# MarbleHE/ABC

Measured on AMD Instinct MI355X. Metric: homomorphic mul+relin/sec, CKKS N=2^14, higher is better.
Workload: dtype u64 (transforms: exact integer arithmetic in f64); 1 GPU; CKKS N=16384, 4 data limbs {50,40,40,40} + special 50-bit prime, ct x ct multiply + relinearize; total_batch=8192, batch_rank0=8192

## Files before the change

abc_amd/csrc/abc_context.hip:

```cpp
#include <cstdlib>
#include <cstring>
#include <mutex>

#include "../../include/abc_hip.h"
#include <dlfcn.h>

#include "abc_context.hpp"
#include "abc_host_math.hpp"
#include "abc_sample.hpp"

namespace abc {

static thread_local std::string g_err;
void set_error(const std::string &msg) { g_err = msg; }

static bool env_on(const char *name) {
  const char *e = std::getenv(name);
  return e && !(e[0] == '0' && e[1] == 0);
}
void read_switches(abc_hip_ctx *c) {
  abc_hip_ctx::Switches s;
  s.no_fused = env_on("ABC_HIP_NO_FUSED");
  s.no_split = env_on("ABC_HIP_NO_SPLIT");
  s.no_split4 = env_on("ABC_HIP_NO_SPLIT4");
  s.no_isplit = env_on("ABC_HIP_NO_ISPLIT");
  s.no_gsplit = env_on("ABC_HIP_NO_GSPLIT");
  s.no_bsplit = env_on("ABC_HIP_NO_BSPLIT");
  s.no_mixed = env_on("ABC_HIP_NO_MIXED");
  s.no_pack = env_on("ABC_HIP_NO_PACK");
  s.no_key_twin = env_on("ABC_HIP_NO_KEY_TWIN");
  s.no_bmul = env_on("ABC_HIP_NO_BMUL");
  s.no_iks = env_on("ABC_HIP_NO_IKS");
  s.no_lean_front = env_on("ABC_HIP_NO_LEAN_FRONT");
  s.no_tensor_intt = env_on("ABC_HIP_NO_TENSOR_INTT");
  s.no_galois_fusion = env_on("ABC_HIP_NO_GALOIS_FUSION");
  s.no_rotate_add_fusion = env_on("ABC_HIP_NO_ROTATE_ADD_FUSION");
  s.no_rotate_mac_fusion = env_on("ABC_HIP_NO_ROTATE_MAC_FUSION");
  s.no_mulplain_rescale_fusion = env_on("ABC_HIP_NO_MULPLAIN_RESCALE_FUSION");
  s.no_tensor_sum = env_on("ABC_HIP_NO_TENSOR_SUM");
  s.main_two_per_cu = env_on("ABC_HIP_MAIN_TWO_PER_CU");
  s.host_sampling = env_on("ABC_HIP_HOST_SAMPLING");
  if (const char *e = std::getenv("ABC_HIP_CHUNK")) s.chunk = (size_t)std::atol(e);
  if (const char *e = std::getenv("ABC_HIP_FEW_LIMBS")) s.few_limbs = (size_t)std::atol(e);
  if (const char *e = std::getenv("ABC_HIP_LEAN_LIMIT")) s.lean_limit = (size_t)std::atol(e);
  if (const char *e = std::getenv("ABC_HIP_PASS0_TARGET_LIMIT")) s.pass0_target_limit = (size_t)std::atol(e);
  if (const char *e = std::getenv("ABC_HIP_BFV_SCRATCH_MB")) s.bfv_scratch_mb = (size_t)std::atol(e);
  if (const char *e = std::getenv("ABC_HIP_LANES")) {
    s.lanes = std::atoi(e);
    if (s.lanes < 1) s.lanes = 1;
    if (s.lanes > abc_hip_ctx::kMaxLanes) s.lanes = abc_hip_ctx::kMaxLanes;
  }
  c->sw = s;
  RouteFacts &f = c->facts;
  f = RouteFacts{};
  f.scheme = c->scheme; f.logn = c->logn; f.K = c->K; f.L = c->L; f.nB = c->nB;
  f.use_fp = c->use_fp; f.behz_fp = c->behz_fp;
  f.big_block_log = big_block_log();
  for (int j = 0; j < c->K; j++) f.bits[j] = (unsigned char)c->h_mods[j].bits;
  f.sw = s;
  f.finish();
}

static Mod make_mod(uint64_t q, int logn, bool ntt) {
  using namespace host;
  Mod m{};
  m.q = q;
  m.two_q = 2 * q;
  const int k = bitlen(q);
  m.bits = (u32)k;
  m.shift = (u32)(k - 1);
  m.mu = (uint64_t)((((u128)1) << (k + 63)) / q);
  m.qd = (double)q;
  m.qinv = 1.0 / (double)q;
  if (ntt) {
    const uint64_t n = 1ull << logn;
    m.inv_n = invmod(n % q, q);
    m.inv_n_s = shoup(m.inv_n, q);
    if (fp_ok(m.bits)) {
      m.inv_n_c = m.inv_n > q / 2 ? -(double)(q - m.inv_n) : (double)m.inv_n;
      m.inv_n_cq = m.inv_n_c / m.qd;
    }
  }
  return m;
}

static void fill_twiddles(uint64_t q, int logn, uint64_t *dst ) {
  using namespace host;
  const size_t n = (size_t)1 << logn;
  const uint64_t psi = min_primitive_root(2 * n, q);
  uint64_t *fwd = dst, *inv = dst + 2 * n;
  uint64_t p = 1;
  for (size_t i = 0; i < n; i++) {
    fwd[2 * (size_t)bitrev((uint32_t)i, logn)] = p;
    p = mulmod(p, psi, q);
  }
  const uint64_t ipsi = invmod(psi, q);
  p = 1;
  for (size_t i = 0; i < n; i++) {
    inv[2 * (size_t)bitrev((uint32_t)i, logn)] = p;
    p = mulmod(p, ipsi, q);
  }
  for (size_t i = 0; i < n; i++) {
    fwd[2 * i + 1] = shoup(fwd[2 * i], q);
    inv[2 * i + 1] = shoup(inv[2 * i], q);
  }
}

static void fill_fp_twiddles(uint64_t q, size_t n, const uint64_t *src , double *dst ) {
  for (size_t i = 0; i < 2 * n; i++) {
    const uint64_t w = src[2 * i];
    dst[i] = w > q / 2 ? -(double)(q - w) : (double)w;
  }
}

static int build_context(abc_hip_ctx *c) {
  using namespace host;
  const int logn = c->logn, K = c->K, L = c->L;
  const size_t N = (size_t)c->n;
  const bool bfv = (c->scheme == ABC_HIP_SCHEME_BFV);
  std::vector<uint64_t> qs(c->primes.begin(), c->primes.begin() + L);
  const uint64_t qsp = c->primes[K - 1];
  DevConst &k = c->h_cst;
  std::memset(&k, 0, sizeof(k));
// ... 1091 lines not shown
```

abc_amd/csrc/abc_kernels_fused.hip:

```cpp
#include <type_traits>

#include "abc_context.hpp"
#include "abc_host_math.hpp"

namespace abc {

template <int LB>
__global__ __launch_bounds__((1 << LB) / 16) void k_fused_tensor_intt(DevCtx c, const u64 *__restrict__ a,
                                                                      const u64 *__restrict__ b, u64 *__restrict__ c01,
                                                                      u64 *__restrict__ c2coef, u64 *__restrict__ c2ntt, int nl) {
  __shared__ u64 lds[lds_words(LB)];
  const int j = blockIdx.x % nl;
  const size_t ct = blockIdx.x / nl;
  const size_t N = (size_t)1 << LB, pw = (size_t)nl * N;
  const Mod m = c.mods[j];
  const NttTable t = ntt_table(c, j);
  const u64 *__restrict__ a0 = a + ct * 2 * pw + j * N, *__restrict__ a1 = a0 + pw;
  const u64 *__restrict__ b0 = b + ct * 2 * pw + j * N, *__restrict__ b1 = b0 + pw;
  u64 *__restrict__ o0 = c01 + ct * 2 * pw + j * N, *__restrict__ o1 = o0 + pw;
  u64 *__restrict__ dcoef = c2coef + (ct * nl + j) * N, *__restrict__ dntt = c2ntt + (ct * nl + j) * N;
  ntt_inv_block<LB>(
      lds,
      [&](int, int i) {
        const u64 x0 = a0[i], x1 = a1[i], y0 = b0[i], y1 = b1[i];
// ... 431 lines not shown
  const int tid = threadIdx.x;
  const int hi0[1] = {0};
  for (int I = 0; I <= nl; I++) {
    if (I == j) continue;
    const int ki = (I == nl) ? c.K - 1 : I;
    const Mod m = mod_at(c, ki);
    const FpTable t = fp_table(c, ki);
    const FpK kk = FpArith::consts(m);
    double y[16];
#pragma unroll
    for (int k = 0; k < 16; k++) y[k] = src[k];
    fwd_pass<FpArith, LB, 0, 4>(y, hi0, t, kk, 0, 0);
    double *__restrict__ dst = part + ((ct * (nl + 1) + I) * nl + j) * (size_t)c.ps;
    store_half_done<LB>(dst, y, tid, kk, (pack && I < nl) ? pack_kind(m.bits) : 0);
  }
}

template <int NL>
__global__ __launch_bounds__(NL ? NL * 64 : 768) void k_split_special_fp(DevCtx c, const double *__restrict__ part, const u64 *__restrict__ key,
                                                                         const double *__restrict__ keyf, double *__restrict__ tsp_half,
                                                                         int nl_rt) {
  extern __shared__ double dyn[];
  const int nl = NL ? NL : nl_rt;
  const int J = __builtin_amdgcn_readfirstlane((int)(threadIdx.x >> 6));
  const int lane = threadIdx.x & 63;
  const int blk = blockIdx.x & 15;
  const size_t ct = (size_t)(blockIdx.x >> 4);
  const size_t N = (size_t)c.n, base = (size_t)blk << 10;
  const int ki = c.K - 1;
  const Mod m = mod_at(c, ki);
  const FpTable t = fp_table(c, ki);
  const double q = m.qd, qinv = m.qinv;
  {
    double *buf = dyn + J * lds_words(10);
    const double *__restrict__ src = part + ((ct * (nl + 1) + nl) * nl + J) * (size_t)c.ps + base;
    ntt_fwd_block_a<10, FpTail>(
        buf, [&](int, int i) { return fp_centre(src[i], q, qinv); }, [&](int, int i, double v) { buf[lds_pad(i)] = v; }, t, m, 4, blk,
        lane);
  }
  __syncthreads();
  for (int e = 2 * (int)threadIdx.x; e < 1024; e += 2 * (int)blockDim.x) {
    double s0[2] = {0.0, 0.0}, s1[2] = {0.0, 0.0};
#pragma unroll
    for (int Jx = 0; Jx < (NL ? NL : 12); Jx++) {
      if (!NL && Jx >= nl) break;
      const f64x2 v = *reinterpret_cast<const f64x2 *>(dyn + Jx * lds_words(10) + lds_pad(e));
      const size_t i0 = (((size_t)Jx * 2 + 0) * c.K + ki) * N + base + e, i1 = i0 + (size_t)c.K * N;
      f64x2 k0, k1;
      if (keyf) {
        k0 = *reinterpret_cast<const f64x2 *>(keyf + i0);
        k1 = *reinterpret_cast<const f64x2 *>(keyf + i1);
      } else {
        const u64x2 r0 = *reinterpret_cast<const u64x2 *>(key + i0), r1 = *reinterpret_cast<const u64x2 *>(key + i1);
        k0.x = fp_from_u64(r0.x); k0.y = fp_from_u64(r0.y);
        k1.x = fp_from_u64(r1.x); k1.y = fp_from_u64(r1.y);
      }
      s0[0] += fp_mulmod(v.x, k0.x, q, qinv);
      s0[1] += fp_mulmod(v.y, k0.y, q, qinv);
      s1[0] += fp_mulmod(v.x, k1.x, q, qinv);
      s1[1] += fp_mulmod(v.y, k1.y, q, qinv);
      if (Jx == 7) {
#pragma unroll
        for (int k = 0; k < 2; k++) {
          s0[k] = fp_centre(s0[k], q, qinv);
          s1[k] = fp_centre(s1[k], q, qinv);
        }
      }
    }
    f64x2 r;
    r.x = fp_centre(s0[0], q, qinv); r.y = fp_centre(s0[1], q, qinv);
    *reinterpret_cast<f64x2 *>(dyn + lds_pad(e)) = r;
    r.x = fp_centre(s1[0], q, qinv); r.y = fp_centre(s1[1], q, qinv);
    *reinterpret_cast<f64x2 *>(dyn + lds_words(10) + lds_pad(e)) = r;
  }
  __syncthreads();
  for (int comp = J; comp < 2; comp += nl) {
    double *buf = dyn + comp * lds_words(10);
    double *__restrict__ dst = tsp_half + (ct * 2 + comp) * (size_t)c.ps + base;
    ntt_inv_block_a<10, FpArith>(
        buf, [&](int, int i) { return buf[lds_pad(i)]; }, [&](int, int i, double v) { dst[i] = v; }, t, m, 4, blk, lane);
  }
}

static void launch_split_special(hipStream_t st, abc_hip_ctx *c, size_t cc, int nl, const double *part, const u64 *key, double *tsp_half) {
  const dim3 grid((unsigned)(cc * 16)), block(64 * nl);
  const size_t lds = (size_t)((nl < 2 ? 2 : nl) * lds_words(10)) * 8;
  const double *keyf = key_twin_lookup(c, key);
#define ABC_SP(NLV) hipLaunchKernelGGL((k_split_special_fp<NLV>), grid, block, lds, st, c->dc, part, key, keyf, tsp_half, nl)
  switch (nl) {
    case 1: ABC_SP(1); break;
    case 2: ABC_SP(2); break;
    case 3: ABC_SP(3); break;
    case 4: ABC_SP(4); break;
    default: ABC_SP(0); break;
  }
#undef ABC_SP
}

struct FusedScratch {
  u64 *coef, *ntt, *dec, *ksacc, *tsp, *tlast, *c01;
};
static inline FusedScratch carve(u64 *base, size_t chunk, int nl, size_t N) {
  FusedScratch s;
  s.coef = base;
  s.ntt = s.coef + chunk * nl * N;
  s.dec = s.ntt + chunk * nl * N;
  s.ksacc = s.dec + chunk * nl * (nl + 1) * N;
  s.tsp = s.ksacc + chunk * 2 * nl * N;
  s.tlast = s.tsp + chunk * 2 * N;
  s.c01 = s.tlast + chunk * 2 * N;
  return s;
}


template <int LB>
__global__ __launch_bounds__(256) void k_split3_pass_fp(DevCtx c, const double *__restrict__ tsp_half, double *__restrict__ tpart, int nl,
                                                        int pack) {
  static_assert(LB == 14, "split transforms are laid out for N = 2^14");
  const size_t cc = blockIdx.x >> 2;
  const int p = (int)((blockIdx.x & 3) << 8) + (int)threadIdx.x;
  const int hi0[1] = {0};
  double x[16];
  {
    const Mod ms = mod_at(c, c.K - 1);
    const FpTable ts = fp_table(c, c.K - 1);
    const FpK ks = FpArith::consts(ms);
    const double *__restrict__ src = tsp_half + cc * (size_t)c.ps;
#pragma unroll
    for (int k = 0; k < 16; k++) x[k] = src[(k << 10) + p];
    FpArith::centre16(x, ks);
    inv_pass<FpArith, LB, 0, 4>(x, hi0, ts, ks, 0, 0);
    const double half = (double)(ms.q >> 1);
#pragma unroll
    for (int k = 0; k < 16; k++) {
      const double w = fp_centre(fp_mul_lazy(x[k], ms.inv_n_c, ms.inv_n_cq, ms.qd) + half, ms.qd, ms.qinv);
      x[k] = w < 0.0 ? w + ms.qd : w;
    }
  }
  const u64 half = c.mods[c.K - 1].q >> 1;
  for (int j = 0; j < nl; j++) {
    const Mod m = mod_at(c, j);
    const FpTable t = fp_table(c, j);
    const FpK kk = FpArith::consts(m);
    const double fix = round_fix<double>(half, m);
    double y[16];
#pragma unroll
    for (int k = 0; k < 16; k++) y[k] = x[k] + fix;
    fwd_pass<FpArith, LB, 0, 4>(y, hi0, t, kk, 0, 0);
    double *__restrict__ dst = tpart + (cc * nl + j) * (size_t)c.ps;
    store_half_done<LB>(dst, y, p, kk, pack ? pack_kind(m.bits) : 0);
  }
}

template <int MODE, bool GAL, int NL, class... A>
__global__ __launch_bounds__(NL ? (NL + 1) * 64 : 832) void k_split3_main_fp(DevCtx c, const double *__restrict__ part,
                                                                              const double *__restrict__ tpart,
                                                                              const u64 *__restrict__ opa, const u64 *__restrict__ opb,
                                                                              size_t opa_stride, size_t opb_stride, int add_c1,
                                                                              const u64 *__restrict__ key, u64 *__restrict__ out, int nl_rt,
                                                                              u32 gelt, AccArg<A>... acc_) {
  constexpr bool ACC = kWithAcc<A...>, MAC = kWithMac<A...>;
  static_assert(!(ACC || MAC) || MODE == 1, "the second addend belongs to the key switch");
  [[maybe_unused]] const u64 *acc = acc_ptr(acc_...);
  [[maybe_unused]] const AccArg<WithMac> mac = mac_arg(acc_...);
  extern __shared__ double dyn[];
  const int nl = NL ? NL : nl_rt;
  const int W = __builtin_amdgcn_readfirstlane((int)(threadIdx.x >> 6));
  const int lane = threadIdx.x & 63;
  const int blk = blockIdx.x & 15;
  const int I = (int)((blockIdx.x >> 4) % nl);
// ... 599 lines not shown
```

abc_amd/csrc/abc_ntt.hpp:

```cpp
#pragma once

#include <type_traits>

#include "abc_modarith.hpp"

namespace abc {

__device__ __forceinline__ int lds_pad(int i) { return i + ((i >> 6) << 2); }
constexpr int lds_words(int lb) { return (1 << lb) + ((1 << lb) >> 6) * 4; }

struct NttTable {
  const u64x2 *tw;
  const u64x2 *itw;
};
struct alignas(16) f64x2 {
  double x, y;
};
#define ABC_CONST_AS __attribute__((address_space(4)))
struct FpTable {
  const ABC_CONST_AS double *tw, *itw;
};
__device__ __forceinline__ double tw_load(const ABC_CONST_AS double *p) { return *p; }
__device__ __forceinline__ u64x2 tw_load(const u64x2 *p) { return *p; }

struct FpK {
  double q, qinv;
  bool red;
};
#pragma clang fp contract(off)
__device__ __forceinline__ double fp_mul_lazy(double y, double w, double wq, double q) {
  const double h = y * w;
  const double l = __builtin_fma(y, w, -h);
  const double c = __builtin_rint(y * wq);
  return __builtin_fma(-c, q, h) + l;
}
__device__ __forceinline__ double fp_mul_tw(double y, double w, double q, double qinv) {
  const double h = y * w;
  const double l = __builtin_fma(y, w, -h);
  const double c = __builtin_rint(h * qinv);
  return __builtin_fma(-c, q, h) + l;
}
__device__ __forceinline__ double fp_mulmod(double x, double y, double q, double qinv) {
  const double h = x * y;
  const double l = __builtin_fma(x, y, -h);
  const double c = __builtin_rint(h * qinv);
  return __builtin_fma(-c, q, h) + l;
}
__device__ __forceinline__ double fp_centre(double x, double q, double qinv) {
  return __builtin_fma(-__builtin_rint(x * qinv), q, x);
}
__device__ __forceinline__ double fp_from_u64(u64 v) {
  return __longlong_as_double((long long)(v | 0x4330000000000000ull)) - 4503599627370496.0;
}
__device__ __forceinline__ u64 fp_to_canon(double x, double q, double qinv) {
  double r = fp_centre(x, q, qinv);
  const u32 neg = (u32)((int)(u32)((u64)__double_as_longlong(r) >> 32) >> 31);
  const u64 qb = (u64)__double_as_longlong(q);
  const u64 add = ((u64)((u32)(qb >> 32) & neg) << 32) | (u64)((u32)qb & neg);
  r += __longlong_as_double((long long)add);
  return (u64)__double_as_longlong(r + 4503599627370496.0) & 0x000fffffffffffffull;
}
__device__ __forceinline__ u64 fp_mac_canon(double x, double p, u64 acc, double q, double qinv) {
  return fp_to_canon(fp_mulmod(fp_centre(x, q, qinv), p, q, qinv) + fp_from_u64(acc), q, qinv);
}
__device__ __forceinline__ u64 fp_to_lazy(double x, double q, double qinv) {
  const double r = fp_centre(x, q, qinv);
  return (u64)__double_as_longlong(r + (4503599627370496.0 + q)) & 0x000fffffffffffffull;
}
__host__ __device__ __forceinline__ bool fp_ok(u32 bits) { return bits <= 50; }

__host__ __device__ __forceinline__ int pack_kind(u32 bits) { return bits <= 40 ? 1 : bits <= 48 ? 2 : 0; }
constexpr double kPackMagic = 6755399441055744.0;
template <int PK>
__device__ __forceinline__ void pack_store(double *limb, size_t n, size_t idx, double centred) {
  const u64 b = (u64)__double_as_longlong(centred + kPackMagic);
  reinterpret_cast<u32 *>(limb)[idx] = (u32)b;
  if (PK == 1) reinterpret_cast<unsigned char *>(limb)[4 * n + idx] = (unsigned char)(b >> 32);
  else reinterpret_cast<unsigned short *>(reinterpret_cast<unsigned char *>(limb) + 4 * n)[idx] = (unsigned short)(b >> 32);
}
template <int PK>
__device__ __forceinline__ u64x2 pack_load_pair(const double *limb, size_t n, size_t idx) {
  u64x2 r;
  r.x = *reinterpret_cast<const u64 *>(reinterpret_cast<const u32 *>(limb) + idx);
  if (PK == 1) r.y = *reinterpret_cast<const unsigned short *>(reinterpret_cast<const unsigned char *>(limb) + 4 * n + idx);
  else r.y = *reinterpret_cast<const u32 *>(reinterpret_cast<const unsigned char *>(limb) + 4 * n + 2 * idx);
  return r;
}
template <int PK>
__device__ __forceinline__ void pack_decode_pair(const u64x2 &r, double &v0, double &v1) {
  const u32 h = (u32)r.y;
  const int h0 = PK == 1 ? (int)(signed char)(h & 0xffu) : (int)(short)(h & 0xffffu);
  const int h1 = PK == 1 ? (int)(signed char)((h >> 8) & 0xffu) : ((int)h >> 16);
  const u64 b0 = ((u64)(u32)(0x43380000 + h0) << 32) | (u32)r.x;
  const u64 b1 = ((u64)(u32)(0x43380000 + h1) << 32) | (u32)(r.x >> 32);
  v0 = __longlong_as_double((long long)b0) - kPackMagic;
  v1 = __longlong_as_double((long long)b1) - kPackMagic;
}

template <int LB> struct Sched;
template <> struct Sched<10> { static constexpr int R0 = 4, R1 = 4, R2 = 2, R3 = 0; };
template <> struct Sched<11> { static constexpr int R0 = 4, R1 = 3, R2 = 2, R3 = 2; };
template <> struct Sched<12> { static constexpr int R0 = 4, R1 = 4, R2 = 2, R3 = 2; };
template <> struct Sched<13> { static constexpr int R0 = 4, R1 = 4, R2 = 3, R3 = 2; };
template <> struct Sched<14> { static constexpr int R0 = 4, R1 = 4, R2 = 4, R3 = 2; };
template <int LB> struct TailSched;
template <> struct TailSched<10> { static constexpr int R0 = 3, R1 = 4, R2 = 3, R3 = 0; };

__device__ __forceinline__ u64 canon4(u64 v, const Mod &m) { return csub(csub(v, m.two_q), m.q); }
__device__ __forceinline__ u64 canon32(u64 v, const Mod &m) {
  v = csub(v, m.two_q << 4);
  v = csub(v, m.two_q << 3);
  v = csub(v, m.two_q << 2);
  v = csub(v, m.two_q << 1);
  return canon4(v, m);
}
template <bool GUARD>
__device__ __forceinline__ u64 canon_fwd(u64 v, const Mod &m) { return GUARD ? canon4(v, m) : canon32(v, m); }
__host__ __device__ __forceinline__ bool unguarded_ok(u32 bits) { return bits <= 57; }
__device__ __forceinline__ u64 scale_inv_n(u64 v, const Mod &m) { return mul_shoup(v, m.inv_n, m.inv_n_s, m.q); }

template <class E = u64>
__device__ __forceinline__ E round_fix(u64 half, const Mod &m) {
  const u64 hm = reduce64(half, m);
  return hm ? (E)(m.q - hm) : (E)0;
}
struct DropInv {
  u64 w, ws;
  double c, cq;
};

template <bool GUARD>
struct IntArith {
  using E = u64;
  using TW = u64x2;
  using Table = NttTable;
  template <int LB> using sched = Sched<LB>;
  struct K {
    u64 q, two_q;
  };
  __device__ __forceinline__ static K consts(const Mod &m) { return K{m.q, m.two_q}; }
  __device__ __forceinline__ static void fwd(E &X, E &Y, const TW tp, const K &k) {
    if (GUARD) {
      const u64 a = csub(X, k.two_q);
      const u64 v = mul_shoup_lazy(Y, tp.x, tp.y, k.q);
      X = a + v;
      Y = a + k.two_q - v;
    } else {
      const u64 a = X;
      const u64 v = mul_shoup_lazy4(Y, tp.x, tp.y, k.q);
      X = a + v;
      Y = a + (k.two_q << 1) - v;
    }
  }
  __device__ __forceinline__ static void inv(E &X, E &Y, const TW tp, const K &k) {
    const u64 a = X, c = Y;
    X = csub(a + c, k.two_q);
    Y = mul_shoup_lazy(a + k.two_q - c, tp.x, tp.y, k.q);
  }
  template <int PASS> __device__ __forceinline__ static void fwd_begin(E (&)[16], const K &) {}
  template <int PASS> __device__ __forceinline__ static void inv_begin(E (&)[16], const K &) {}
  __device__ __forceinline__ static E from_u64(u64 v) { return v; }
  __device__ __forceinline__ static E mul_u64(u64 a, u64 b, const Mod &m) { return mul_mod(a, b, m); }
  __device__ __forceinline__ static bool fwd_accepts(u64 q_from, const Mod &m) { return GUARD ? q_from <= m.q : (q_from >> 3) < m.q; }
  template <bool LAZY> __device__ __forceinline__ static u64 fwd_out(E v, const Mod &m) { return LAZY ? v : canon_fwd<GUARD>(v, m); }
  __device__ __forceinline__ static E scale_n(E v, const Mod &m) { return scale_inv_n(v, m); }
  __device__ __forceinline__ static u64 canon(E r, const Mod &) { return r; }
  __device__ __forceinline__ static u64 canon_add(E r, E c, const Mod &m) { return add_mod(r, c, m.q); }
  __device__ __forceinline__ static E reduce_fix(u64 t, E fix, const Mod &m) { return add_mod(reduce64(t, m), fix, m.q); }
  __device__ __forceinline__ static E diff_mul_fwd(E x, E y, const DropInv &d, const Mod &m) {
    return mul_shoup(GUARD ? sub_mod(x, canon4(y, m), m.q) : x + (m.two_q << 5) - y, d.w, d.ws, m.q);
  }
};

struct FpArith {
  using E = double;
  using TW = double;
  using Table = FpTable;
  using K = FpK;
  template <int LB> using sched = Sched<LB>;
  __device__ __forceinline__ static K consts(const Mod &m) { return K{m.qd, m.qinv, m.bits >= 49}; }
  __device__ __forceinline__ static void fwd(E &X, E &Y, const TW w, const K &k) {
    const double a = X;
    const double v = fp_mul_tw(Y, w, k.q, k.qinv);
    X = a + v;
    Y = a - v;
  }
  __device__ __forceinline__ static void inv(E &X, E &Y, const TW w, const K &k) {
    const double a = X, c = Y;
    X = a + c;
    Y = fp_mul_tw(a - c, w, k.q, k.qinv);
  }
  __device__ __forceinline__ static void centre16(E (&x)[16], const K &k) {
#pragma unroll
    for (int r = 0; r < 16; r++) x[r] = fp_centre(x[r], k.q, k.qinv);
  }
  template <int PASS> __device__ __forceinline__ static void fwd_begin(E (&x)[16], const K &k) {
    if (PASS > 0 && k.red) centre16(x, k);
  }
  template <int PASS> __device__ __forceinline__ static void inv_begin(E (&x)[16], const K &k) {
    if (PASS > 0 || k.red) centre16(x, k);
  }
  __device__ __forceinline__ static E from_u64(u64 v) { return fp_from_u64(v); }
  __device__ __forceinline__ static E mul_u64(u64 a, u64 b, const Mod &m) { return fp_mulmod(fp_from_u64(a), fp_from_u64(b), m.qd, m.qinv); }
  __device__ __forceinline__ static bool fwd_accepts(u64, const Mod &) { return true; }
  template <bool LAZY> __device__ __forceinline__ static u64 fwd_out(E v, const Mod &m) { return fp_to_lazy(v, m.qd, m.qinv); }
  __device__ __forceinline__ static E scale_n(E v, const Mod &m) { return fp_mul_lazy(v, m.inv_n_c, m.inv_n_cq, m.qd); }
  __device__ __forceinline__ static u64 canon(E r, const Mod &m) { return fp_to_canon(r, m.qd, m.qinv); }
  __device__ __forceinline__ static u64 canon_add(E r, E c, const Mod &m) { return fp_to_canon(r + c, m.qd, m.qinv); }
  __device__ __forceinline__ static E reduce_fix(u64 t, E fix, const Mod &m) { return fp_from_u64(t) + fix; }
  __device__ __forceinline__ static E diff_mul_fwd(E x, E y, const DropInv &d, const Mod &m) { return fp_mul_lazy(x - y, d.c, d.cq, m.qd); }
};

struct FpTail : FpArith {
  template <int LB> using sched = TailSched<LB>;
  template <int PASS> __device__ __forceinline__ static void fwd_begin(E (&x)[16], const K &k) {
    if (PASS == 2 && k.red && k.q >= 562949953421312.0) centre16(x, k);
  }
};

template <class A, int LB, int S, int R>
__device__ __forceinline__ void fwd_pass(typename A::E (&x)[16], const int (&hi)[16 >> R], const typename A::Table &t,
                                         const typename A::K &kk, int S0, int b) {
  constexpr int NG = 16 >> R;
#pragma unroll
  for (int u = 0; u < R; u++) {
    const int half = 1 << (R - 1 - u);
#pragma unroll
    for (int g = 0; g < NG; g++) {
      int base = (1 << (S0 + S + u)) + (b << (S + u)) + (hi[g] << u);
#pragma unroll
      for (int k = 0; k < (1 << R); k++) {
        if (k & half) continue;
        int idx = base + (k >> (R - u));
        A::fwd(x[g * (1 << R) + k], x[g * (1 << R) + (k | half)], tw_load(t.tw + idx), kk);
      }
    }
  }
}

template <class A, int LB, int S, int R>
__device__ __forceinline__ void fwd_pass_lds(typename A::E (&x)[16], const int (&hi)[16 >> R], const typename A::TW *ltw,
                                             const typename A::K &kk) {
  constexpr int NG = 16 >> R;
#pragma unroll
  for (int u = 0; u < R; u++) {
    const int half = 1 << (R - 1 - u);
#pragma unroll
    for (int g = 0; g < NG; g++) {
      int base = (1 << (S + u)) + (hi[g] << u);
#pragma unroll
      for (int k = 0; k < (1 << R); k++) {
        if (k & half) continue;
        int idx = base + (k >> (R - u));
        A::fwd(x[g * (1 << R) + k], x[g * (1 << R) + (k | half)], ltw[idx], kk);
      }
    }
  }
}
template <int LB, class TW, int PER>
__device__ __forceinline__ void block_twiddles_fetch(const ABC_CONST_AS TW *tw, int S0, int b, int tid, int nthreads, TW (&v)[PER]) {
#pragma unroll
  for (int r = 0; r < PER; r++) {
    int mm = tid + r * nthreads;
    if (mm < 1) mm = 1;
    if (mm > (1 << LB) - 1) mm = (1 << LB) - 1;
    const int sl = 31 - __builtin_clz(mm);
    v[r] = tw_load(tw + (((1 << S0) + b) << sl) + (mm - (1 << sl)));
  }
}
template <int LB, class TW, int PER>
__device__ __forceinline__ void block_twiddles_fetch(const TW *tw, int S0, int b, int tid, int nthreads, TW (&v)[PER]) {
#pragma unroll
  for (int r = 0; r < PER; r++) {
    int mm = tid + r * nthreads;
    if (mm < 1) mm = 1;
    if (mm > (1 << LB) - 1) mm = (1 << LB) - 1;
    const int sl = 31 - __builtin_clz(mm);
    v[r] = tw[(((1 << S0) + b) << sl) + (mm - (1 << sl))];
  }
}
template <int LB, class TW, int PER>
__device__ __forceinline__ void block_twiddles_store(TW *ltw, int tid, int nthreads, const TW (&v)[PER]) {
#pragma unroll
  for (int r = 0; r < PER; r++) {
    const int mm = tid + r * nthreads;
    if (mm >= 1 && mm < (1 << LB)) ltw[mm] = v[r];
  }
}

template <class A, int LB, int S, int R>
__device__ __forceinline__ void inv_pass(typename A::E (&x)[16], const int (&hi)[16 >> R], const typename A::Table &t,
                                         const typename A::K &kk, int S0, int b) {
  constexpr int NG = 16 >> R;
#pragma unroll
  for (int u = R - 1; u >= 0; u--) {
    const int half = 1 << (R - 1 - u);
#pragma unroll
    for (int g = 0; g < NG; g++) {
      int base = (1 << (S0 + S + u)) + (b << (S + u)) + (hi[g] << u);
#pragma unroll
      for (int k = 0; k < (1 << R); k++) {
        if (k & half) continue;
        int idx = base + (k >> (R - u));
        A::inv(x[g * (1 << R) + k], x[g * (1 << R) + (k | half)], tw_load(t.itw + idx), kk);
      }
    }
  }
}

template <class A, int LB, int S, int R>
__device__ __forceinline__ void inv_pass_lds(typename A::E (&x)[16], const int (&hi)[16 >> R], const typename A::TW *ltw,
                                             const typename A::K &kk) {
  constexpr int NG = 16 >> R;
#pragma unroll
  for (int u = R - 1; u >= 0; u--) {
    const int half = 1 << (R - 1 - u);
#pragma unroll
    for (int g = 0; g < NG; g++) {
      int base = (1 << (S + u)) + (hi[g] << u);
#pragma unroll
      for (int k = 0; k < (1 << R); k++) {
        if (k & half) continue;
        int idx = base + (k >> (R - u));
        A::inv(x[g * (1 << R) + k], x[g * (1 << R) + (k | half)], ltw[idx], kk);
      }
    }
  }
}

template <int R>
__device__ __forceinline__ void fwd_cross(double (&x)[1 << R], const FpTable &t, const FpK &kk) {
#pragma unroll
  for (int u = 0; u < R; u++) {
    const int half = 1 << (R - 1 - u);
#pragma unroll
    for (int k = 0; k < (1 << R); k++) {
      if (k & half) continue;
      FpArith::fwd(x[k], x[k | half], tw_load(t.tw + (1 << u) + (k >> (R - u))), kk);
    }
  }
}
template <int R>
__device__ __forceinline__ void inv_cross(double (&x)[1 << R], const FpTable &t, const FpK &kk) {
#pragma unroll
  for (int u = R - 1; u >= 0; u--) {
    const int half = 1 << (R - 1 - u);
#pragma unroll
    for (int k = 0; k < (1 << R); k++) {
      if (k & half) continue;
      FpArith::inv(x[k], x[k | half], tw_load(t.itw + (1 << u) + (k >> (R - u))), kk);
    }
    if (R > 4 && u == R - 4) {
#pragma unroll
      for (int k = 0; k < (1 << R); k++) x[k] = fp_centre(x[k], kk.q, kk.qinv);
    }
  }
}

template <int LB, int S, int R>
struct PassIdx {
  static constexpr int T = (1 << LB) / 16;
  static constexpr int NG = 16 >> R;
  static constexpr int LOGG = LB - S - R;
  static constexpr int G = 1 << LOGG;
  static constexpr bool UNIFORM = (G >= 64);
  __device__ __forceinline__ static void groups(int tid, int (&hi)[NG], int (&lo)[NG]) {
    const int wave = __builtin_amdgcn_readfirstlane(tid >> 6);
    const int lane = tid & 63;
#pragma unroll
    for (int g = 0; g < NG; g++) {
      if (UNIFORM) {
        const int pw = wave * (64 * NG) + g * 64;
        hi[g] = pw >> LOGG;
        lo[g] = (pw + lane) & (G - 1);
      } else {
        const int p = wave * (64 * NG) + g * 64 + lane;
// ... 153 lines not shown
}

template <int LB, bool GUARD = true, class Load, class Store>
__device__ __forceinline__ void ntt_fwd_block(u64 *lds, Load load, Store store, const NttTable &t, const Mod &m, int S0,
                                              int b) {
  ntt_fwd_block_a<LB, IntArith<GUARD>>(lds, load, store, t, m, S0, b);
}

template <int LB, class A, class Load, class Store, bool LTW = false>
__device__ __forceinline__ void ntt_inv_block_a(typename A::E *lds, Load load, Store store, const typename A::Table &t,
                                                const Mod &m, int S0, int b, int tid_in = -1,
                                                const typename A::TW *ltw = nullptr ) {
  using SC = Sched<LB>;
  const int tid = tid_in < 0 ? (int)threadIdx.x : tid_in;
  const typename A::K kk = A::consts(m);
  typename A::E x[16];
  constexpr int SA = SC::R0, SB = SC::R0 + SC::R1, SCc = SC::R0 + SC::R1 + SC::R2;
  if constexpr (SC::R3 != 0) {
    constexpr int S = SCc, R = SC::R3;
    using P = PassIdx<LB, S, R>;
    int hi[P::NG], lo[P::NG];
    P::groups(tid, hi, lo);
#pragma unroll
    for (int g = 0; g < P::NG; g++)
#pragma unroll
      for (int k = 0; k < (1 << R); k++) x[g * (1 << R) + k] = load(g * (1 << R) + k, P::elem(hi[g], lo[g], k));
    A::template inv_begin<0>(x, kk);
    if constexpr (LTW && !P::UNIFORM) inv_pass_lds<A, LB, S, R>(x, hi, ltw, kk);
    else inv_pass<A, LB, S, R>(x, hi, t, kk, S0, b);
    lds_store<LB, S, R>(lds, x, hi, lo);
    wave_sync();
  }
  {
    constexpr int S = SB, R = SC::R2;
    using P = PassIdx<LB, S, R>;
    int hi[P::NG], lo[P::NG];
    P::groups(tid, hi, lo);
    if constexpr (SC::R3 != 0) {
      lds_load<LB, S, R>(lds, x, hi, lo);
    } else {
#pragma unroll
      for (int g = 0; g < P::NG; g++)
#pragma unroll
        for (int k = 0; k < (1 << R); k++) x[g * (1 << R) + k] = load(g * (1 << R) + k, P::elem(hi[g], lo[g], k));
    }
    A::template inv_begin<(SC::R3 != 0 ? 1 : 0)>(x, kk);
    if constexpr (LTW && !P::UNIFORM) inv_pass_lds<A, LB, S, R>(x, hi, ltw, kk);
    else inv_pass<A, LB, S, R>(x, hi, t, kk, S0, b);
    lds_store<LB, S, R>(lds, x, hi, lo);
    wave_sync();
  }
  {
    constexpr int S = SA, R = SC::R1;
    using P = PassIdx<LB, S, R>;
    int hi[P::NG], lo[P::NG];
    P::groups(tid, hi, lo);
    lds_load<LB, S, R>(lds, x, hi, lo);
    A::template inv_begin<(SC::R3 != 0 ? 2 : 1)>(x, kk);
    if constexpr (LTW && !P::UNIFORM) inv_pass_lds<A, LB, S, R>(x, hi, ltw, kk);
    else inv_pass<A, LB, S, R>(x, hi, t, kk, S0, b);
    lds_store<LB, S, R>(lds, x, hi, lo);
    if constexpr (LB <= 10) wave_sync(); else block_sync_lds();
  }
  {
    constexpr int S = 0, R = SC::R0;
    using P = PassIdx<LB, S, R>;
    int hi[P::NG], lo[P::NG];
    P::groups(tid, hi, lo);
    lds_load<LB, S, R>(lds, x, hi, lo);
    A::template inv_begin<(SC::R3 != 0 ? 3 : 2)>(x, kk);
    if constexpr (LTW && !P::UNIFORM) inv_pass_lds<A, LB, S, R>(x, hi, ltw, kk);
    else inv_pass<A, LB, S, R>(x, hi, t, kk, S0, b);
#pragma unroll
    for (int g = 0; g < P::NG; g++)
#pragma unroll
      for (int k = 0; k < (1 << R); k++) store(g * (1 << R) + k, P::elem(hi[g], lo[g], k), x[g * (1 << R) + k]);
  }
}

template <int LB, class Load, class Store>
__device__ __forceinline__ void ntt_inv_block(u64 *lds, Load load, Store store, const NttTable &t, const Mod &m, int S0,
                                              int b) {
  ntt_inv_block_a<LB, IntArith<true>>(lds, load, store, t, m, S0, b);
}

template <int LB, class A, bool MUL = false>
__device__ __forceinline__ void divround_to_coef(typename A::E *lds, const Mod m, const typename A::Table t,
                                                 const u64 *__restrict__ src, u64 *__restrict__ dst,
                                                 const u64 *__restrict__ pl = nullptr) {
  using E = typename A::E;
  const E half = (E)(m.q >> 1);
  ntt_inv_block_a<LB, A>(
      lds,
      [&](int, int i) {
        if constexpr (MUL) return A::mul_u64(src[i], pl[i], m);
        else return A::from_u64(src[i]);
      },
      [&](int, int i, E v) { dst[i] = A::canon_add(A::scale_n(v, m), half, m); }, t, m, 0, 0);
}
template <int LB, class A, bool REDUCE, bool ADD, bool MUL = false>
__device__ __forceinline__ void divround_finish(typename A::E *lds, const Mod m, const typename A::Table t,
                                                const std::conditional_t<REDUCE, u64, typename A::E> fix, const DropInv d,
                                                const u64 *__restrict__ tl, const u64 *__restrict__ x, const u64 *__restrict__ cin,
                                                u64 *__restrict__ o, const u64 *__restrict__ pl = nullptr) {
  using E = typename A::E;
  ntt_fwd_block_a<LB, A>(
      lds,
      [&](int, int i) {
        if constexpr (REDUCE) return A::from_u64(IntArith<true>::reduce_fix(tl[i], fix, m));
        else return A::reduce_fix(tl[i], fix, m);
      },
      [&](int, int i, E v) {
        E xi;
        if constexpr (MUL) xi = A::mul_u64(x[i], pl[i], m);
        else xi = A::from_u64(x[i]);
        const E r = A::diff_mul_fwd(xi, v, d, m);
        if constexpr (ADD) o[i] = A::canon_add(r, A::from_u64(cin[i]), m);
        else o[i] = A::canon(r, m);
      },
      t, m, 0, 0);
}

}
```

abc_amd/csrc/abc_route.hpp:

```cpp
#pragma once

#include <cstddef>
#include <cstdint>
#include <cstdio>

namespace abc {

struct Switches {
  bool no_fused = false, no_split = false, no_split4 = false, no_isplit = false, no_gsplit = false, no_lean_front = false, no_bsplit = false, no_mixed = false, no_pack = false, no_key_twin = false, no_bmul = false, no_iks = false, no_tensor_intt = false;
  bool no_galois_fusion = false;
  bool no_rotate_add_fusion = false;
  bool no_rotate_mac_fusion = false;
  bool no_mulplain_rescale_fusion = false;
  bool no_tensor_sum = false;
  bool main_two_per_cu = false;
  bool host_sampling = false;
  size_t chunk = 0, few_limbs = 48, lean_limit = 96, bfv_scratch_mb = 0, pass0_target_limit = 128;
  int lanes = 2;
};

constexpr unsigned kFpBits = 50;
constexpr unsigned kLazyBits = 55;
constexpr unsigned kUnguardedBits = 57;
constexpr unsigned kIsplitBits = 60;

constexpr size_t fused_scratch_limbs(int nl) { return (size_t)nl * (nl + 1) + 6 * (size_t)nl + 4; }

struct RouteFacts {
  int scheme = 0, logn = 0, K = 0, L = 0, nB = 0;
  bool use_fp = true, behz_fp = false;
  int big_block_log = 12;
  unsigned char bits[17] = {};
  Switches sw;
  unsigned widest = 0;
  uint32_t fp_mask = 0;
  bool all_fp = false;
  bool guard = false;
  bool lazy = false;
  void finish() {
    widest = 0;
    fp_mask = 0;
    for (int j = 0; j < K; j++) {
      if (bits[j] > widest) widest = bits[j];
      if (bits[j] <= kFpBits) fp_mask |= 1u << j;
    }
    all_fp = use_fp && widest <= kFpBits;
    guard = widest > kUnguardedBits;
    lazy = widest <= kLazyBits;
  }
  uint32_t fp_data_mask(int nl) const { return fp_mask & ((1u << nl) - 1u); }
  bool data_fp(int nl) const { return fp_data_mask(nl) == (1u << nl) - 1u; }
  bool special_fp() const { return K > 0 && ((fp_mask >> (K - 1)) & 1u); }
};

enum class Seq {
  split14,
  gsplit15,
  isplit,
  bsplit14,
  bsplit_big,
  lds_fp,
  lds_int,
  bmul,
  generic
};
enum class KsFront { plain, fp, iks };
enum class BfvMul { behz, split, big };
enum class Rescale { generic, fp, mixed };

struct KsRoute {
  Seq seq;
  KsFront front;
};
struct MulRoute {
  Seq seq;
  BfvMul mul;
  KsRoute ks;
};
struct RotRoute {
  bool fold;
  KsRoute ks;
};
struct RotTailRoute {
  RotRoute rot;
  bool fused;
};
using RotAddRoute = RotTailRoute;
using RotMacRoute = RotTailRoute;
struct RescaleRoute {
  Rescale kind;
  uint32_t fpmask;
};
struct MulPlainRescaleRoute {
  RescaleRoute rescale;
  bool fused;
};
struct MulSumRoute {
  KsRoute ks;
// ... 96 lines not shown
  return {rot, rot.fold && seq_takes_acc(f, rot.ks, nl) && !in_place && !f.sw.no_rotate_add_fusion};
}

inline RotTailRoute route_rotate_mac(const RouteFacts &f, int nl, bool in_place) {
  const RotRoute rot = route_rotate(f, nl, false);
  return {rot, rot.fold && seq_takes_plain(f, rot.ks, nl) && !in_place && !f.sw.no_rotate_mac_fusion};
}

inline RescaleRoute route_rescale(const RouteFacts &f, int nl, bool in_place) {
  if (f.logn > 14 || f.logn < 10 || in_place || f.sw.no_fused) return {Rescale::generic, 0u};
  if (f.use_fp && f.data_fp(nl)) return {Rescale::fp, 0u};
  if (f.sw.no_isplit) return {Rescale::generic, 0u};
  return {Rescale::mixed, (f.use_fp && !f.sw.no_mixed) ? f.fp_data_mask(nl) : 0u};
}

inline MulPlainRescaleRoute route_mulplain_rescale(const RouteFacts &f, int nl) {
  const RescaleRoute r = route_rescale(f, nl, false);
  return {r, r.kind != Rescale::generic && !f.sw.no_mulplain_rescale_fusion};
}

inline MulSumRoute route_mul_sum(const RouteFacts &f, int nl) {
  return {route_keyswitch(f, nl), f.scheme == 2 && !f.sw.no_tensor_sum};
}

struct ChunkPlan {
  size_t chunk;
  int lanes;
};
inline ChunkPlan plan_chunks(const RouteFacts &f, int nl, size_t count) {
  ChunkPlan p{f.sw.chunk, f.sw.lanes};
  if (count <= 8) p.lanes = 1;
  if (!p.chunk) {
    const size_t per_ct_bytes = fused_scratch_limbs(nl) * ((size_t)1 << f.logn) * 8;
    const size_t cap = ((size_t)4 << 30) / per_ct_bytes / (size_t)p.lanes;
    p.chunk = (count + p.lanes - 1) / p.lanes;
    if (p.chunk > 128) p.chunk = 128;
    if (p.chunk > cap) p.chunk = cap;
    if (p.chunk < 1) p.chunk = 1;
  }
  if (p.chunk > count) p.chunk = count;
  return p;
}
inline size_t mul_sum_group(const RouteFacts &f, int nl, size_t count) {
  const ChunkPlan p = plan_chunks(f, nl, count);
  const size_t unit = p.chunk * (size_t)p.lanes;
  if (f.sw.chunk || unit >= count) return unit < count ? unit : count;
  const size_t per_ct_bytes = 3 * (size_t)nl * ((size_t)1 << f.logn) * 8;
  const size_t units = ((size_t)4 << 30) / per_ct_bytes / unit;
  const size_t group = unit * (units ? units : 1);
  return group < count ? group : count;
}
struct ChunkRoute {
  bool lean = false;
  bool pack = false;
  bool main4 = false;
  bool per_target = false;
  bool guard = false, lazy = false;
  bool fp_twin = false;
  uint32_t fpmask = 0;
};
inline ChunkRoute route_chunk(const RouteFacts &f, Seq seq, int nl, size_t cc) {
  ChunkRoute k;
  switch (seq) {
    case Seq::split14:
      k.lean = !f.sw.no_lean_front && cc * nl <= f.sw.lean_limit;
      k.main4 = !f.sw.no_split4 && nl >= 1 && nl <= 5;
      k.pack = k.main4 && !f.sw.no_pack;
      break;
    case Seq::bsplit14: k.per_target = cc * nl < f.sw.pass0_target_limit; break;
    case Seq::lds_int:
      k.guard = f.guard;
      k.lazy = f.lazy;
      break;
    case Seq::isplit:
      k.guard = f.guard;
      k.fp_twin = f.logn == 14 && !f.sw.no_mixed;
      k.fpmask = (f.use_fp && !f.sw.no_mixed) ? f.fp_data_mask(nl) : 0u;
      break;
    default: break;
  }
  return k;
}

inline const char *name(Seq s) {
  constexpr const char *names[] = {"split14", "gsplit15", "isplit", "bsplit14", "bsplit_big", "lds_fp", "lds_int", "bmul", "generic"};
  return names[(int)s];
}
inline const char *name(KsFront k) { return k == KsFront::fp ? "fp" : k == KsFront::iks ? "iks" : "plain"; }
inline const char *name(BfvMul m) { return m == BfvMul::split ? "bmul" : m == BfvMul::big ? "bmul_big" : "behz"; }
inline const char *name(Rescale r) { return r == Rescale::fp ? "fp" : r == Rescale::mixed ? "mixed" : "generic"; }

inline void format_ks(char *buf, size_t cap, const RouteFacts &f, const KsRoute &r, int nl, size_t count) {
  const ChunkRoute k = route_chunk(f, r.seq, nl, plan_chunks(f, nl, count).chunk);
  switch (r.seq) {
    case Seq::split14: snprintf(buf, cap, "split14 front=%s pack=%d main=%s", k.lean ? "lean" : "fat", (int)k.pack, k.main4 ? "split4" : "split3"); break;
    case Seq::isplit: snprintf(buf, cap, "isplit%d guard=%d fpmask=0x%x", f.logn, (int)k.guard, (unsigned)k.fpmask); break;
    case Seq::bsplit14: snprintf(buf, cap, "bsplit14 pass0=%s", k.per_target ? "per_target" : "per_limb"); break;
    case Seq::lds_int: snprintf(buf, cap, "lds_int guard=%d lazy=%d", (int)k.guard, (int)k.lazy); break;
    case Seq::generic:
      if (r.front == KsFront::iks) snprintf(buf, cap, "generic front=iks guard=%d", (int)f.guard);
      else snprintf(buf, cap, "generic front=%s", name(r.front));
      break;
    default: snprintf(buf, cap, "%s", name(r.seq)); break;
  }
}
enum RouteOp { kRouteMulRelin = 0, kRouteKeyswitch = 1, kRouteRotate = 2, kRouteRescale = 3, kRouteMultiply = 4, kRouteRotateAdd = 5, kRouteRotateMacPlain = 7, kRouteMulPlainRescale = 10, kRouteMulSumRelin = 12 };
inline int format_op(char *buf, size_t cap, const RouteFacts &f, int op, int nl, size_t count, bool in_place) {
  char ks[80];
  int n = -2;
  if (op == kRouteMulRelin) {
    const MulRoute r = route_mul_relin(f, nl);
    format_ks(ks, sizeof ks, f, r.seq == Seq::generic ? r.ks : KsRoute{r.seq, KsFront::plain}, nl, count);
    n = r.seq == Seq::generic ? snprintf(buf, cap, "generic mul=%s ks=%s", f.scheme == 2 ? "tensor" : name(r.mul), ks) : snprintf(buf, cap, "%s", ks);
  } else if (op == kRouteKeyswitch) {
    format_ks(ks, sizeof ks, f, route_keyswitch(f, nl), nl, count);
    n = snprintf(buf, cap, "%s", ks);
  } else if (op == kRouteRotate) {
    const RotRoute r = route_rotate(f, nl, in_place);
    format_ks(ks, sizeof ks, f, r.ks, nl, count);
    n = snprintf(buf, cap, "%s %s", r.fold ? "fold" : "permute", ks);
  } else if (op == kRouteRotateAdd) {
    const RotTailRoute r = route_rotate_add(f, nl, in_place);
    format_ks(ks, sizeof ks, f, r.rot.ks, nl, count);
    n = r.fused ? snprintf(buf, cap, "fold+add %s", ks) : snprintf(buf, cap, "%s add=separate %s", r.rot.fold ? "fold" : "permute", ks);
  } else if (op == kRouteRotateMacPlain) {
    const RotTailRoute r = route_rotate_mac(f, nl, in_place);
    format_ks(ks, sizeof ks, f, r.rot.ks, nl, count);
    n = r.fused ? snprintf(buf, cap, "fold+mac %s", ks) : snprintf(buf, cap, "%s mac=separate %s", r.rot.fold ? "fold" : "permute", ks);
  } else if (op == kRouteRescale) {
    const RescaleRoute r = route_rescale(f, nl, in_place);
    n = r.kind == Rescale::mixed ? snprintf(buf, cap, "mixed fpmask=0x%x", (unsigned)r.fpmask) : snprintf(buf, cap, "%s", name(r.kind));
  } else if (op == kRouteMulPlainRescale) {
    const MulPlainRescaleRoute r = route_mulplain_rescale(f, nl);
    const char *how = r.fused ? "fused" : "separate";
    n = r.rescale.kind == Rescale::mixed ? snprintf(buf, cap, "mixed fpmask=0x%x mulplain=%s", (unsigned)r.rescale.fpmask, how)
                                         : snprintf(buf, cap, "%s mulplain=%s", name(r.rescale.kind), how);
  } else if (op == kRouteMulSumRelin) {
    const MulSumRoute r = route_mul_sum(f, nl);
    format_ks(ks, sizeof ks, f, r.ks, nl, mul_sum_group(f, nl, count));
    n = snprintf(buf, cap, "%s tensor=%s", ks, r.sum ? "sum" : "per_term");
  } else if (op == kRouteMultiply) {
    n = snprintf(buf, cap, "%s", f.scheme == 1 ? name(route_bfv_multiply(f)) : "tensor");
  }
  return n < 0 ? n : (size_t)n < cap ? n : -1;
}

}
```

Baseline: 435,900 mul+relin/s.

## Use two wavefronts per digit with radix-8 tail NTT in special-prime keyswitch kernel

Adds a new special-prime split kernel that assigns 128 threads (two wavefronts) per digit instead of 64. Each lane now handles 8 elements with three radix-8 passes plus a radix-2 pass, where the old kernel used 16 elements per lane. The forward NTT, key multiply-accumulate and inverse NTT are reorganised across the two waves, with extra block-level LDS syncs. This is meant to raise parallelism and lower register pressure per lane, at the cost of more synchronisation. It is on by default for nl<=4, and an env switch restores the old kernel.

```diff
diff --git a/abc_amd/csrc/abc_context.hip b/abc_amd/csrc/abc_context.hip
--- a/abc_amd/csrc/abc_context.hip
+++ b/abc_amd/csrc/abc_context.hip
@@ -39,6 +39,7 @@
   s.no_mulplain_rescale_fusion = env_on("ABC_HIP_NO_MULPLAIN_RESCALE_FUSION");
   s.no_tensor_sum = env_on("ABC_HIP_NO_TENSOR_SUM");
   s.main_two_per_cu = env_on("ABC_HIP_MAIN_TWO_PER_CU");
+  s.special_one_wave = env_on("ABC_HIP_SPECIAL_ONE_WAVE");
   s.host_sampling = env_on("ABC_HIP_HOST_SAMPLING");
   if (const char *e = std::getenv("ABC_HIP_CHUNK")) s.chunk = (size_t)std::atol(e);
   if (const char *e = std::getenv("ABC_HIP_FEW_LIMBS")) s.few_limbs = (size_t)std::atol(e);
diff --git a/abc_amd/csrc/abc_kernels_fused.hip b/abc_amd/csrc/abc_kernels_fused.hip
--- a/abc_amd/csrc/abc_kernels_fused.hip
+++ b/abc_amd/csrc/abc_kernels_fused.hip
@@ -537,10 +537,96 @@
   }
 }
 
+template <int NL>
+__global__ __launch_bounds__(NL * 128, NL == 3 ? 6 : 8) void k_split_special_x8_fp(DevCtx c, const double *__restrict__ part, const u64 *__restrict__ key,
+                                                                    const double *__restrict__ keyf, double *__restrict__ tsp_half) {
+  static_assert(NL >= 1 && NL <= 4, "two wavefronts per digit, eight wavefronts");
+  extern __shared__ double dyn[];
+  constexpr int nl = NL;
+  const int J = __builtin_amdgcn_readfirstlane((int)(threadIdx.x >> 7));
+  const int t128 = threadIdx.x & 127;
+  const int blk = blockIdx.x & 15;
+  const size_t ct = (size_t)(blockIdx.x >> 4);
+  const size_t N = (size_t)c.n, base = (size_t)blk << 10;
+  const int ki = c.K - 1;
+  const Mod m = mod_at(c, ki);
+  const FpTable t = fp_table(c, ki);
+  const FpK kk = FpArith::consts(m);
+  const double q = m.qd, qinv = m.qinv;
+  double raw[8];
+  {
+    const double *__restrict__ src = part + ((ct * (nl + 1) + nl) * nl + J) * (size_t)c.ps + base;
+#pragma unroll
+    for (int k = 0; k < 8; k++) raw[k] = src[(k << 7) + t128];
+  }
+  u64x2 kw[NL];
+  auto load_keys = [&](int e, int comp) {
+    const u64 *kp = (keyf ? reinterpret_cast<const u64 *>(keyf) : key) + ((size_t)comp * c.K + ki) * N + base;
+    const size_t digit = 2 * (size_t)c.K * N;
+#pragma unroll
+    for (int Jx = 0; Jx < NL; Jx++)
+      kw[Jx] = *reinterpret_cast<const u64x2 *>(reinterpret_cast<const char *>(kp + Jx * digit) + (unsigned)e * 8u);
+  };
+  ntt_fwd_tail1024_x8<FpTail8>(
+      dyn + J * lds_words(10), [&](int k, int) { return fp_centre(raw[k], q, qinv); }, t, m, 4, blk, t128);
+  block_sync_lds();
+  auto pairs = [&](auto TWIN) {
+    for (int e = 2 * (int)threadIdx.x; e < 1024; e += 2 * 128 * NL) {
+      const int ti = tail8_pair_twiddle(4, blk, e);
+      const double wf = tw_load(t.tw + ti), wi = tw_load(t.itw + ti);
+      load_keys(e, 0);
+      auto word = [](u64 w) { return decltype(TWIN)::value ? __longlong_as_double((long long)w) : fp_from_u64(w); };
+      f64x2 v[NL];
+#pragma unroll
+      for (int Jx = 0; Jx < NL; Jx++) {
+        v[Jx] = *reinterpret_cast<const f64x2 *>(dyn + Jx * lds_words(10) + lds_pad(e));
+        FpTail8::fwd(v[Jx].x, v[Jx].y, wf, kk);
+      }
+#pragma unroll
+      for (int comp = 0; comp < 2; comp++) {
+        if (comp) load_keys(e, 1);
+        f64x2 r = {0.0, 0.0};
+#pragma unroll
+        for (int Jx = 0; Jx < NL; Jx++) {
+          r.x += fp_mulmod(v[Jx].x, word(kw[Jx].x), q, qinv);
+          r.y += fp_mulmod(v[Jx].y, word(kw[Jx].y), q, qinv);
+        }
+        r.x = fp_centre(r.x, q, qinv); r.y = fp_centre(r.y, q, qinv);
+        FpTail8::inv(r.x, r.y, wi, kk);
+        *reinterpret_cast<f64x2 *>(dyn + comp * lds_words(10) + lds_pad(e)) = r;
+      }
+    }
+  };
+  if (keyf) pairs(std::true_type{});
+  else pairs(std::false_type{});
+  block_sync_lds();
+  int ti128 = t128;
+  asm volatile("" : "+v"(ti128));
+  for (int c0 = 0; c0 < 2; c0 += nl) {
+    const int comp = c0 + J;
+    double *buf = dyn + (comp & 1) * lds_words(10);
+    if (comp < 2) ntt_inv_tail1024_x8_local<FpTail8>(buf, t, m, 4, blk, ti128);
+    block_sync_lds();
+    if (comp < 2) {
+      double *__restrict__ dst = tsp_half + (ct * 2 + comp) * (size_t)c.ps + base;
+      ntt_inv_tail1024_x8_cross<FpTail8>(
+          buf, [&](int, int i, double v) { dst[i] = v; }, t, m, 4, blk, ti128);
+    }
+  }
+}
+
 static void launch_split_special(hipStream_t st, abc_hip_ctx *c, size_t cc, int nl, const double *part, const u64 *key, double *tsp_half) {
-  const dim3 grid((unsigned)(cc * 16)), block(64 * nl);
   const size_t lds = (size_t)((nl < 2 ? 2 : nl) * lds_words(10)) * 8;
   const double *keyf = key_twin_lookup(c, key);
+  if (special_two_waves(c->facts, nl)) {
+    const dim3 grid((unsigned)(cc * 16)), block(128 * nl);
+    dispatch_nl<1, 4>(nl, [&](auto NL) {
+      hipLaunchKernelGGL((k_split_special_x8_fp<decltype(NL)::value>), grid, block, lds, st, c->dc, part, key, keyf,
+                         tsp_half);
+    });
+    return;
+  }
+  const dim3 grid((unsigned)(cc * 16)), block(64 * nl);
 #define ABC_SP(NLV) hipLaunchKernelGGL((k_split_special_fp<NLV>), grid, block, lds, st, c->dc, part, key, keyf, tsp_half, nl)
   switch (nl) {
     case 1: ABC_SP(1); break;
diff --git a/abc_amd/csrc/abc_ntt.hpp b/abc_amd/csrc/abc_ntt.hpp
--- a/abc_amd/csrc/abc_ntt.hpp
+++ b/abc_amd/csrc/abc_ntt.hpp
@@ -105,6 +105,8 @@
 template <> struct Sched<14> { static constexpr int R0 = 4, R1 = 4, R2 = 4, R3 = 2; };
 template <int LB> struct TailSched;
 template <> struct TailSched<10> { static constexpr int R0 = 3, R1 = 4, R2 = 3, R3 = 0; };
+template <int LB> struct Tail8Sched;
+template <> struct Tail8Sched<10> { static constexpr int R0 = 3, R1 = 3, R2 = 3, R3 = 1; };
 
 __device__ __forceinline__ u64 canon4(u64 v, const Mod &m) { return csub(csub(v, m.two_q), m.q); }
 __device__ __forceinline__ u64 canon32(u64 v, const Mod &m) {
@@ -217,11 +219,26 @@
     if (PASS == 2 && k.red && k.q >= 562949953421312.0) centre16(x, k);
   }
 };
-
-template <class A, int LB, int S, int R>
-__device__ __forceinline__ void fwd_pass(typename A::E (&x)[16], const int (&hi)[16 >> R], const typename A::Table &t,
+struct FpTail8 : FpArith {
+  template <int LB> using sched = Tail8Sched<LB>;
+  template <int PASS> __device__ __forceinline__ static void fwd_begin(E (&x)[8], const K &k) {
+    if (PASS == 2 && k.red && k.q >= 562949953421312.0) {
+#pragma unroll
+      for (int r = 0; r < 8; r++) x[r] = fp_centre(x[r], k.q, k.qinv);
+    }
+  }
+  template <int PASS> __device__ __forceinline__ static void inv_begin(E (&x)[8], const K &k) {
+    if (PASS >= 2) {
+#pragma unroll
+      for (int r = 0; r < 8; r++) x[r] = fp_centre(x[r], k.q, k.qinv);
+    }
+  }
+};
+
+template <class A, int LB, int S, int R, int W = 16>
+__device__ __forceinline__ void fwd_pass(typename A::E (&x)[W], const int (&hi)[W >> R], const typename A::Table &t,
                                          const typename A::K &kk, int S0, int b) {
-  constexpr int NG = 16 >> R;
+  constexpr int NG = W >> R;
 #pragma unroll
   for (int u = 0; u < R; u++) {
     const int half = 1 << (R - 1 - u);
@@ -288,10 +305,10 @@
   }
 }
 
-template <class A, int LB, int S, int R>
-__device__ __forceinline__ void inv_pass(typename A::E (&x)[16], const int (&hi)[16 >> R], const typename A::Table &t,
+template <class A, int LB, int S, int R, int W = 16>
+__device__ __forceinline__ void inv_pass(typename A::E (&x)[W], const int (&hi)[W >> R], const typename A::Table &t,
                                          const typename A::K &kk, int S0, int b) {
-  constexpr int NG = 16 >> R;
+  constexpr int NG = W >> R;
 #pragma unroll
   for (int u = R - 1; u >= 0; u--) {
     const int half = 1 << (R - 1 - u);
@@ -611,6 +628,95 @@
 __device__ __forceinline__ void ntt_inv_block(u64 *lds, Load load, Store store, const NttTable &t, const Mod &m, int S0,
                                               int b) {
   ntt_inv_block_a<LB, IntArith<true>>(lds, load, store, t, m, S0, b);
+}
+
+struct Tail8Idx {
+  __device__ __forceinline__ static int row1(int t) { return ((t >> 6) << 2) | ((t >> 5) & 1) | ((t >> 3) & 2); }
+  __device__ __forceinline__ static int hi2(int t) {
+    return ((t >> 6) << 5) | (((t >> 5) & 1) << 4) | (((t >> 1) & 3) << 2) | (((t >> 4) & 1) << 1) | ((t >> 3) & 1);
+  }
+};
+template <class A, class Load>
+__device__ __forceinline__ void ntt_fwd_tail1024_x8(typename A::E *lds, Load load, const typename A::Table &t, const Mod &m, int S0, int b,
+                                                    int t128) {
+  constexpr int LB = 10;
+  using SC = typename A::template sched<LB>;
+  static_assert(SC::R0 == 3 && SC::R1 == 3 && SC::R2 == 3 && SC::R3 == 1, "one radix-8 group per lane and pass");
+  const typename A::K kk = A::consts(m);
+  typename A::E x[8];
+  {
+    const int hi[1] = {0};
+#pragma unroll
+    for (int k = 0; k < 8; k++) x[k] = load(k, (k << 7) + t128);
+    fwd_pass<A, LB, 0, 3>(x, hi, t, kk, S0, b);
+#pragma unroll
+    for (int k = 0; k < 8; k++) lds[lds_pad((k << 7) + t128)] = x[k];
+  }
+  block_sync_lds();
+  {
+    const int hi[1] = {Tail8Idx::row1(t128)};
+    const int at = (hi[0] << 7) + (t128 & 15);
+#pragma unroll
+    for (int k = 0; k < 8; k++) x[k] = lds[lds_pad(at + (k << 4))];
+    A::template fwd_begin<1>(x, kk);
+    fwd_pass<A, LB, 3, 3>(x, hi, t, kk, S0, b);
+#pragma unroll
+    for (int k = 0; k < 8; k++) lds[lds_pad(at + (k << 4))] = x[k];
+  }
+  wave_sync();
+  {
+    const int hi[1] = {Tail8Idx::hi2(t128)};
+    const int at = (hi[0] << 4) + (t128 & 1);
+#pragma unroll
+    for (int k = 0; k < 8; k++) x[k] = lds[lds_pad(at + (k << 1))];
+    A::template fwd_begin<2>(x, kk);
+    fwd_pass<A, LB, 6, 3>(x, hi, t, kk, S0, b);
+#pragma unroll
+    for (int k = 0; k < 8; k++) lds[lds_pad(at + (k << 1))] = x[k];
+  }
+}
+__device__ __forceinline__ int tail8_pair_twiddle(int S0, int b, int e) { return (1 << (S0 + 9)) + (b << 9) + (e >> 1); }
+template <class A>
+__device__ __forceinline__ void ntt_inv_tail1024_x8_local(typename A::E *lds, const typename A::Table &t, const Mod &m, int S0, int b,
+                                                          int t128) {
+  constexpr int LB = 10;
+  const typename A::K kk = A::consts(m);
+  typename A::E x[8];
+  {
+    const int hi[1] = {Tail8Idx::hi2(t128)};
+    const int at = (hi[0] << 4) + (t128 & 1);
+#pragma unroll
+    for (int k = 0; k < 8; k++) x[k] = lds[lds_pad(at + (k << 1))];
+    A::template inv_begin<1>(x, kk);
+    inv_pass<A, LB, 6, 3>(x, hi, t, kk, S0, b);
+#pragma unroll
+    for (int k = 0; k < 8; k++) lds[lds_pad(at + (k << 1))] = x[k];
+  }
+  wave_sync();
+  {
+    const int hi[1] = {Tail8Idx::row1(t128)};
+    const int at = (hi[0] << 7) + (t128 & 15);
+#pragma unroll
+    for (int k = 0; k < 8; k++) x[k] = lds[lds_pad(at + (k << 4))];
+    A::template inv_begin<2>(x, kk);
+    inv_pass<A, LB, 3, 3>(x, hi, t, kk, S0, b);
+#pragma unroll
+    for (int k = 0; k < 8; k++) lds[lds_pad(at + (k << 4))] = x[k];
+  }
+}
+template <class A, class Store>
+__device__ __forceinline__ void ntt_inv_tail1024_x8_cross(const typename A::E *lds, Store store, const typename A::Table &t, const Mod &m,
+                                                          int S0, int b, int t128) {
+  constexpr int LB = 10;
+  const typename A::K kk = A::consts(m);
+  typename A::E x[8];
+  const int hi[1] = {0};
+#pragma unroll
+  for (int k = 0; k < 8; k++) x[k] = lds[lds_pad((k << 7) + t128)];
+  A::template inv_begin<3>(x, kk);
+  inv_pass<A, LB, 0, 3>(x, hi, t, kk, S0, b);
+#pragma unroll
+  for (int k = 0; k < 8; k++) store(k, (k << 7) + t128, x[k]);
 }
 
 template <int LB, class A, bool MUL = false>
diff --git a/abc_amd/csrc/abc_route.hpp b/abc_amd/csrc/abc_route.hpp
--- a/abc_amd/csrc/abc_route.hpp
+++ b/abc_amd/csrc/abc_route.hpp
@@ -14,6 +14,7 @@
   bool no_mulplain_rescale_fusion = false;
   bool no_tensor_sum = false;
   bool main_two_per_cu = false;
+  bool special_one_wave = false;
   bool host_sampling = false;
   size_t chunk = 0, few_limbs = 48, lean_limit = 96, bfv_scratch_mb = 0, pass0_target_limit = 128;
   int lanes = 2;
@@ -276,6 +277,8 @@
   return k;
 }
 
+inline bool special_two_waves(const RouteFacts &f, int nl) { return nl >= 1 && nl <= 4 && !f.sw.special_one_wave; }
+
 inline const char *name(Seq s) {
   constexpr const char *names[] = {"split14", "gsplit15", "isplit", "bsplit14", "bsplit_big", "lds_fp", "lds_int", "bmul", "generic"};
   return names[(int)s];
@@ -287,7 +290,10 @@
 inline void format_ks(char *buf, size_t cap, const RouteFacts &f, const KsRoute &r, int nl, size_t count) {
   const ChunkRoute k = route_chunk(f, r.seq, nl, plan_chunks(f, nl, count).chunk);
   switch (r.seq) {
-    case Seq::split14: snprintf(buf, cap, "split14 front=%s pack=%d main=%s", k.lean ? "lean" : "fat", (int)k.pack, k.main4 ? "split4" : "split3"); break;
+    case Seq::split14:
+      snprintf(buf, cap, "split14 front=%s pack=%d main=%s%s", k.lean ? "lean" : "fat", (int)k.pack, k.main4 ? "split4" : "split3",
+               (f.sw.special_one_wave && nl <= 4) ? " special=one_wave" : "");
+      break;
     case Seq::isplit: snprintf(buf, cap, "isplit%d guard=%d fpmask=0x%x", f.logn, (int)k.guard, (unsigned)k.fpmask); break;
     case Seq::bsplit14: snprintf(buf, cap, "bsplit14 pass0=%s", k.per_target ? "per_target" : "per_limb"); break;
     case Seq::lds_int: snprintf(buf, cap, "lds_int guard=%d lazy=%d", (int)k.guard, (int)k.lazy); break;
```

Measured after the change: 440,400 mul+relin/s (median of 6 runs). Within noise of the previous version (+1.0%).
